# nv-legate/legate.sparse

Hardware: AMD Instinct MI355X
Metric: cg_iters_per_sec (higher is better)
Workload: dtype fp64; 1 GPU; model=poisson2d-5pt-cg, nx=16384, n=268435456, nnz=1342111744, parallelism=dp1 1-D row partition + window gather

## Files before the change

sparse/kernels/__init__.py:

```python
from __future__ import annotations

import os

import torch

_EXT = None
_TRIED = False

_DIR = os.path.dirname(os.path.abspath(__file__))
BUILD_DIR = os.path.join(_DIR, "_build")
SO_PATH = os.path.join(BUILD_DIR, "sparse_hip.so")


def ext():
    global _EXT, _TRIED
    if _EXT is not None or _TRIED:
        return _EXT
    _TRIED = True
    if os.path.exists(SO_PATH):
        torch.ops.load_library(SO_PATH)
        _EXT = torch.ops.sparse_hip
    return _EXT


# ... 324 lines not shown
                     ts._level_ptr, ts._sched, b, x)


def ilu0_factor(fac, values, flag):
    ls = fac._Ls
    ext().ilu0_factor(fac._indptr, fac._indices, values, fac._diag_ptr,
                      ls._order, ls._level_ptr, fac._sched, flag)


_DIA_CONST_DTYPES = (torch.float32, torch.float64)


class DiaMirror:

    __slots__ = ("dvals", "offs", "W", "m", "row0", "off_min", "off_max",
                 "cvals", "mask", "adj")

    def __init__(self, dvals, offs, W, m, row0, off_min=0, off_max=0,
                 cvals=None, mask=None, adj=0):
        self.adj = adj
        self.off_min = off_min
        self.off_max = off_max
        self.dvals = dvals
        self.offs = offs
        self.W = W
        self.m = m
        self.row0 = row0
        self.cvals = cvals
        self.mask = mask

    @property
    def compressed(self) -> bool:
        return self.mask is not None

    def source(self):
        if self.compressed:
            return self.cvals, self.mask
        return self.dvals, None


def build_dia(A, row0: int, compress: bool = True):
    m = A.nrows
    if m == 0 or A.nnz == 0:
        return None
    counts = A.indptr[1:] - A.indptr[:-1]
    rows = torch.repeat_interleave(
        torch.arange(row0, row0 + m, dtype=torch.int64, device=A.device), counts)
    diag = A.indices.long() - rows
    CH = 1 << 30
    if diag.numel() <= CH:
        offs = torch.unique(diag)
    else:
        parts = [torch.unique(diag[i: i + CH])
                 for i in range(0, diag.numel(), CH)]
        offs = torch.unique(torch.cat(parts))
    W = int(offs.numel())
    mp = (m + 1) // 2 * 2
    if W == 0 or W > 48 or W * mp > 1.6 * A.nnz + 4096:
        return None
    need = W * mp * A.values.element_size()
    free, _t = torch.cuda.mem_get_info(A.values.device)
    if need > 0.5 * free:
        return None
    dvals = torch.zeros(W * mp, dtype=A.values.dtype, device=A.device)
    ext().build_dia(A.indptr, A.indices, A.values, offs.contiguous(), dvals,
                    W, int(row0))
    cvals = mask = None
    if (compress and W <= 32 and dvals.dtype in _DIA_CONST_DTYPES
            and os.environ.get("SPARSE_DIA_NOCOMPRESS") != "1"):
        cvals = torch.zeros(W, dtype=dvals.dtype, device=A.device)
        mdt = (torch.uint8 if W <= 8 else
               torch.uint16 if W <= 16 else torch.uint32)
        mask = torch.empty(mp, dtype=mdt, device=A.device)
        ok = torch.ones(1, dtype=torch.int32, device=A.device)
        ext().dia_classify(dvals, cvals, mask, ok, W)
        if int(ok.item()):
            dvals = None
        else:
            cvals = mask = None
    ho = offs.tolist()
    adj = sum(1 << i for i in range(min(W, 32) - 1) if ho[i + 1] == ho[i] + 1)
    return DiaMirror(dvals, offs, W, m, row0, off_min=ho[0], off_max=ho[-1],
                     cvals=cvals, mask=mask, adj=adj)


def _pieces(p):
    hlo, own, hhi = p
    return hlo.contiguous(), own.contiguous(), hhi.contiguous()


def dia_spmv(dm: DiaMirror, pieces, y, col_lo: int, wsize: int,
             rbase: int = 0, rhi: int = -1):
    ext().dia_spmv(*dm.source(), dm.offs, *_pieces(pieces), y, dm.W, dm.m,
                   int(col_lo), dm.row0, int(wsize), int(rbase), int(rhi),
                   dm.adj)


def dia_spmv_dot(dm: DiaMirror, pieces, y, p, col_lo: int, wsize: int,
                 rbase: int = 0, rhi: int = -1):
    return ext().dia_spmv_dot(*dm.source(), dm.offs, *_pieces(pieces), y, p,
                              dm.W, dm.m, int(col_lo), dm.row0, int(wsize),
                              int(rbase), int(rhi), dm.adj)


def dia_spmv_bpdot(dm: DiaMirror, r_pieces, p_pieces, pnew, q,
                   beta_num, beta_den, col_lo: int, wsize: int):
    return ext().dia_spmv_bpdot(*dm.source(), dm.offs, *_pieces(r_pieces),
                                *_pieces(p_pieces), pnew, q, beta_num,
                                beta_den, dm.W, dm.m, int(col_lo), dm.row0,
                                int(wsize), dm.adj)


def cg_xr_norm2(x, p, r, q, a, b, *, nt: int = -1):
    n = x.numel()
    if n == 0:
        return torch.zeros((), dtype=x.dtype, device=x.device)
    ept = max(1, 16 // x.element_size())
    blocks = (n // ept + 255) // 256 + 1
    partial = torch.empty(blocks, dtype=x.dtype, device=x.device)
    ext().cg_xr_norm2(x, p, r, q, a.to(x.dtype), b.to(x.dtype), partial,
                      int(nt))
    return partial.sum()


def dia_residual(dm: DiaMirror, pieces, b, y, col_lo: int, wsize: int,
                 rbase: int = 0, rhi: int = -1):
    ext().dia_residual(*dm.source(), dm.offs, *_pieces(pieces), b, y, dm.W,
                       dm.m, int(col_lo), dm.row0, int(wsize), int(rbase),
                       int(rhi), dm.adj)


def dia_jacobi(dm: DiaMirror, pieces, xloc, b, dinv, omega, xout,
               col_lo: int, wsize: int, rbase: int = 0, rhi: int = -1):
    ext().dia_jacobi(*dm.source(), dm.offs, *_pieces(pieces), xloc, b, dinv,
                     xout, dm.W, dm.m, int(col_lo), dm.row0, int(wsize),
                     float(omega), int(rbase), int(rhi), dm.adj)


class BsrMirror:

    __slots__ = ("bptr", "bcol", "bvals", "nbrows", "m", "fill")

    def __init__(self, bptr, bcol, bvals, nbrows, m, fill):
        self.bptr = bptr
        self.bcol = bcol
        self.bvals = bvals
        self.nbrows = nbrows
        self.m = m
        self.fill = fill


# ... 118 lines not shown
```

sparse/kernels/src/ops.cpp:

```cpp
#include <algorithm>

#include <torch/library.h>

#include <ATen/ATen.h>

void spmv_hip(at::Tensor, at::Tensor, at::Tensor, at::Tensor, at::Tensor,
              int64_t, double);
void spmv_dot_hip(at::Tensor, at::Tensor, at::Tensor, at::Tensor, at::Tensor,
                  at::Tensor, at::Tensor, int64_t);
void axpby_norm2_hip(at::Tensor, at::Tensor, at::Tensor, at::Tensor, bool,
                     bool, at::Tensor);
void build_ell_hip(at::Tensor, at::Tensor, at::Tensor, at::Tensor, at::Tensor,
                   int64_t, int64_t);
void build_dia_hip(at::Tensor, at::Tensor, at::Tensor, at::Tensor, at::Tensor,
                   int64_t, int64_t);
void ell_spmv_plain_hip(at::Tensor, at::Tensor, at::Tensor, at::Tensor,
                        at::Tensor, at::Tensor, int64_t, int64_t, int64_t,
                        int64_t, int64_t);
at::Tensor ell_spmv_dot_hip(at::Tensor, at::Tensor, at::Tensor, at::Tensor,
                            at::Tensor, at::Tensor, at::Tensor, int64_t,
                            int64_t, int64_t, int64_t, int64_t);
void ell_jacobi_hip(at::Tensor, at::Tensor, at::Tensor, at::Tensor,
                    at::Tensor, at::Tensor, at::Tensor, at::Tensor,
                    at::Tensor, int64_t, int64_t, int64_t, double);
void cg_xr_norm2_hip(at::Tensor, at::Tensor, at::Tensor, at::Tensor,
                     at::Tensor, at::Tensor, at::Tensor, int64_t);
using OptTensor = c10::optional<at::Tensor>;
void dia_classify_hip(at::Tensor, at::Tensor, at::Tensor, at::Tensor, int64_t);
at::Tensor dia_spmv_bpdot_hip(at::Tensor, OptTensor, at::Tensor, at::Tensor,
                              at::Tensor, at::Tensor, at::Tensor, at::Tensor,
                              at::Tensor, at::Tensor, at::Tensor, at::Tensor,
                              at::Tensor, int64_t, int64_t, int64_t, int64_t,
                              int64_t, int64_t);
void dia_spmv_plain_hip(at::Tensor, OptTensor, at::Tensor, at::Tensor,
                        at::Tensor, at::Tensor, at::Tensor, int64_t, int64_t,
                        int64_t, int64_t, int64_t, int64_t, int64_t, int64_t);
at::Tensor dia_spmv_dot_hip(at::Tensor, OptTensor, at::Tensor, at::Tensor,
                            at::Tensor, at::Tensor, at::Tensor, at::Tensor,
                            int64_t, int64_t, int64_t, int64_t, int64_t,
                            int64_t, int64_t, int64_t);
void dia_residual_hip(at::Tensor, OptTensor, at::Tensor, at::Tensor,
                      at::Tensor, at::Tensor, at::Tensor, at::Tensor, int64_t,
                      int64_t, int64_t, int64_t, int64_t, int64_t, int64_t,
                      int64_t);
void dia_jacobi_hip(at::Tensor, OptTensor, at::Tensor, at::Tensor, at::Tensor,
                    at::Tensor, at::Tensor, at::Tensor, at::Tensor,
                    at::Tensor, int64_t, int64_t, int64_t, int64_t, int64_t,
                    double, int64_t, int64_t, int64_t);
void add_nnz_hip(at::Tensor, at::Tensor, at::Tensor, at::Tensor, at::Tensor);
void add_compute_hip(at::Tensor, at::Tensor, at::Tensor, at::Tensor, at::Tensor,
                     at::Tensor, at::Tensor, at::Tensor, at::Tensor, double,
                     double);
void mult_nnz_hip(at::Tensor, at::Tensor, at::Tensor, at::Tensor, at::Tensor);
void mult_compute_hip(at::Tensor, at::Tensor, at::Tensor, at::Tensor,
                      at::Tensor, at::Tensor, at::Tensor, at::Tensor,
                      at::Tensor);
void mult_dense_hip(at::Tensor, at::Tensor, at::Tensor, at::Tensor, at::Tensor);
void axpby_hip(at::Tensor, at::Tensor, at::Tensor, at::Tensor, bool, bool,
               int64_t);
void spmm_hip(at::Tensor, at::Tensor, at::Tensor, at::Tensor, at::Tensor,
              int64_t);
void rspmm_hip(at::Tensor, at::Tensor, at::Tensor, at::Tensor, at::Tensor);
void bsr_spmm_hip(at::Tensor, at::Tensor, at::Tensor, at::Tensor, at::Tensor,
// ... 142 lines not shown
        "Tensor(a!) eidx, Tensor(b!) evals, int W, int pad_idx) -> ()");
  m.def("build_dia(Tensor indptr, Tensor indices, Tensor values, "
        "Tensor offs, Tensor(a!) dvals, int W, int row0) -> ()");
  m.def("ell_spmv(Tensor eidx, Tensor evals, Tensor hlo, Tensor own, "
        "Tensor hhi, Tensor(a!) y, int W, int m, int col_lo, "
        "int rbase, int rhi) -> ()");
  m.def("ell_spmv_dot(Tensor eidx, Tensor evals, Tensor hlo, Tensor own, "
        "Tensor hhi, Tensor(a!) y, Tensor pvec, int W, int m, int col_lo, "
        "int rbase, int rhi) -> Tensor");
  m.def("ell_jacobi(Tensor eidx, Tensor evals, Tensor hlo, Tensor own, "
        "Tensor hhi, Tensor xloc, Tensor b, Tensor dinv, Tensor(a!) xout, "
        "int W, int m, int col_lo, float omega) -> ()");
  m.def("cg_xr_norm2(Tensor(a!) x, Tensor p, Tensor(b!) r, Tensor q, "
        "Tensor a, Tensor b, Tensor(c!) dot_out, int nt=-1) -> ()");
  m.def("dia_classify(Tensor dvals, Tensor(a!) cvals, Tensor(b!) mask, "
        "Tensor(c!) ok, int W) -> ()");
  m.def("dia_spmv_bpdot(Tensor planes, Tensor? mask, Tensor offs, "
        "Tensor r_hlo, Tensor r_own, "
        "Tensor r_hhi, Tensor p_hlo, Tensor p_own, Tensor p_hhi, "
        "Tensor(a!) pnew, Tensor(b!) q, Tensor beta_num, Tensor beta_den, "
        "int W, int m, int col_lo, int row0, int wsize, int adj=0) "
        "-> Tensor");
  m.def("dia_spmv(Tensor planes, Tensor? mask, Tensor offs, Tensor hlo, "
        "Tensor own, "
        "Tensor hhi, Tensor(a!) y, int W, int m, int col_lo, int row0, "
        "int wsize, int rbase, int rhi, int adj=0) -> ()");
  m.def("dia_spmv_dot(Tensor planes, Tensor? mask, Tensor offs, Tensor hlo, "
        "Tensor own, "
        "Tensor hhi, Tensor(a!) y, Tensor pvec, int W, int m, int col_lo, "
        "int row0, int wsize, int rbase, int rhi, int adj=0) -> Tensor");
  m.def("dia_residual(Tensor planes, Tensor? mask, Tensor offs, Tensor hlo, "
        "Tensor own, "
        "Tensor hhi, Tensor b, Tensor(a!) y, int W, int m, int col_lo, "
        "int row0, int wsize, int rbase, int rhi, int adj=0) -> ()");
  m.def("dia_jacobi(Tensor planes, Tensor? mask, Tensor offs, Tensor hlo, "
        "Tensor own, "
        "Tensor hhi, Tensor xloc, Tensor b, Tensor dinv, Tensor(a!) xout, "
        "int W, int m, int col_lo, int row0, int wsize, float omega, "
        "int rbase, int rhi, int adj=0) -> ()");
  m.def("spmm(Tensor indptr, Tensor indices, Tensor vals, Tensor B, "
        "Tensor(a!) C, int col_lo) -> ()");
  m.def("rspmm(Tensor indptr, Tensor indices, Tensor vals, Tensor A, "
        "Tensor(a!) C) -> ()");
  m.def("bsr_spmm(Tensor bptr, Tensor bcol, Tensor bvals, Tensor B, "
        "Tensor(a!) C, int col_lo) -> ()");
  m.def("sddmm(Tensor indptr, Tensor indices, Tensor vals, Tensor C, "
        "Tensor D, Tensor(a!) out, int col_lo) -> ()");
  m.def("csr_to_dense(Tensor indptr, Tensor indices, Tensor vals, "
        "Tensor(a!) out) -> ()");
  m.def("coo_to_csr(Tensor rows, Tensor cols, Tensor vals, Tensor(a!) cursor, "
        "Tensor indptr, Tensor(b!) out_idx, Tensor(c!) out_vals, "
        "Tensor(d!) flags) -> ()");
  m.def("dense_to_csr(Tensor D, Tensor(a!) indptr_or_counts, "
        "Tensor(b!) indices, Tensor(c!) vals, bool fill) -> ()");
// ... 70 lines not shown
```

sparse/kernels/src/spmv.hip:

```cpp
#include <type_traits>

#include "common.h"

namespace {

constexpr int BLK = 256;
constexpr int VT = 8;
constexpr int64_t NNZ_PER_BLOCK = (int64_t)BLK * VT;

template <typename U>
struct alignas(4 * sizeof(U) <= 16 ? 4 * sizeof(U) : 16) Quad {
  U v[4];
};

template <typename U>
struct alignas(2 * sizeof(U) <= 16 ? 2 * sizeof(U) : 16) Pair {
  U a, b;
};

template <typename T>
__device__ __forceinline__ void block_reduce_sum(T* red, int tid) {
  __syncthreads();
  for (int w = BLK / 2; w > 0; w >>= 1) {
    if (tid < w) red[tid] += red[tid + w];
// ... 284 lines not shown
  const int64_t r = (int64_t)blockIdx.x * blockDim.x + threadIdx.x;
  if (r >= mp) return;
  uint32_t word = 0;
  bool same = true;
  for (int k = 0; k < W; ++k) {
    const B b = dbits[(int64_t)k * mp + r];
    if (b != 0) {
      word |= 1u << k;
      same = same && b == cbits[k];
    }
  }
  mask[r] = (M)word;
  if (!same && *ok != 0) *ok = 0;
}



template <typename T>
struct XWindow {
  const T* hlo;
  const T* own;
  const T* hhi;
  int64_t nlo, nown, wsize;

  template <bool SINGLE>
  __device__ __forceinline__ T at(int64_t idx) const {
    if (SINGLE) return own[idx];
    if (idx < nlo) return hlo[idx];
    idx -= nlo;
    if (idx < nown) return own[idx];
// ... 77 lines not shown
  __device__ __forceinline__ Rows rows(int64_t r0) const {
    return {dvals + r0, mp};
  }
};

template <int BYTES> struct UIntOf;
template <> struct UIntOf<2> { using type = uint16_t; };
template <> struct UIntOf<4> { using type = uint32_t; };
template <> struct UIntOf<8> { using type = uint64_t; };

template <typename T, typename M>
struct DiaConstPlanes {
  static constexpr int kBatch = 8;
  const T* __restrict__ cvals;
  const M* __restrict__ mask;

  struct Rows {
    const T* __restrict__ c;
    uint32_t m0, m1;
    __device__ __forceinline__ void at(int k, T& v0, T& v1) const {
      const T ck = c[k];
      const uint32_t bit = 1u << k;
      v0 = (m0 & bit) ? ck : T(0);
      v1 = (m1 & bit) ? ck : T(0);
    }
  };
  __device__ __forceinline__ Rows rows(int64_t r0) const {
    using M2 = typename UIntOf<2 * sizeof(M)>::type;
    const M2 w = nt_load(reinterpret_cast<const M2*>(&mask[r0]));
    return {cvals, (uint32_t)(M)w, (uint32_t)(w >> (8 * sizeof(M)))};
// ... 238 lines not shown
  static constexpr int start = ADJ ? __builtin_ctz(ADJ) : 0;
  static constexpr int len = ADJ ? __builtin_popcount(ADJ) + 1 : 1;
  static_assert(ADJ == 0 || (ADJ >> start) + 1 == (1u << (len - 1)),
                "the adjacent diagonals must form one run");
  __host__ __device__ static constexpr DiaSrc src(int P, int i) {
    const int q = i - start;
    if (ADJ == 0 || P < 0 || q < 0 || q >= len) return kDiaLoad;
    if (((P + q) & 1) == 0) return kDiaLoadAligned;
    return q > 0 ? kDiaFromLo : kDiaFromHi;
  }
  __host__ __device__ static constexpr bool two(int P, int i) {
    return src(P, i) == kDiaFromHi && len >= 3;
  }
};

template <int WC, int R, int NWIN, uint32_t ADJ, int P, typename T,
          typename M, typename Comb, typename Pre, typename Post>
__device__ __forceinline__ void dia_const_interior(
    const DiaConstPlanes<T, M>& planes, const int64_t* __restrict__ offs,
    int W, const T* const* own, Comb comb, bool ctr, int64_t rb,
    int64_t cb, int64_t (&o)[WC ? WC : 8], T (&c)[WC ? WC : 8], Pre pre,
    Post post) {
  constexpr int KB = WC ? WC : 8;
  using Run = DiaRun<ADJ>;
  using M2 = typename UIntOf<2 * sizeof(M)>::type;
  const int64_t t2 = 2 * (int64_t)threadIdx.x;
  const int lane = threadIdx.x & 63;
  M2 mw[R];
#pragma unroll
  for (int j = 0; j < R; ++j) {
    mw[j] = nt_load(
        reinterpret_cast<const M2*>(planes.mask + rb + t2 + j * 2 * BLK));
  }
  T a[R][2];
  Pair<T> cx[R];
#pragma unroll
  for (int j = 0; j < R; ++j) {
    a[j][0] = a[j][1] = ZeroOf<T>::value();
    cx[j] = Pair<T>{T(0), T(0)};
  }
  for (int k0 = 0; k0 < W; k0 += KB) {
    if (k0 > 0) {
#pragma unroll
      for (int i = 0; i < KB; ++i) {
        if (k0 + i < W) {
          o[i] = offs[k0 + i];
          c[i] = planes.cvals[k0 + i];
// ... 94 lines not shown
    post(j, rb + t2 + j * 2 * BLK, a[j][0], a[j][1], true, ctr, cx[j]);
  }
}

template <int WC, int R, bool SINGLE, int NWIN, uint32_t ADJ, typename T,
          typename M, typename Comb, typename Pre, typename Post>
__device__ __forceinline__ void dia_const_rows(
    const DiaConstPlanes<T, M>& planes, const int64_t* __restrict__ offs,
    int Wrt, const XWindow<T>& win0, const XWindow<T>& win1, Comb comb,
    const T* rowvec, int64_t m, int64_t row0, int64_t col_lo, int64_t rbase,
    int64_t rhi, Pre pre, Post post) {
  constexpr int KB = WC ? WC : 8;
  constexpr int64_t S = 2 * (int64_t)BLK * R;
  static_assert(ADJ == 0 || (WC > 0 && (ADJ >> (KB - 1)) == 0),
                "a plan needs a compile-time W");
  using Run = DiaRun<ADJ>;
  const int W = WC ? WC : Wrt;
  const int64_t lim = min(m, rhi);
  const int64_t rb = rbase + (int64_t)blockIdx.x * S;
  const int64_t cb = row0 + rb - col_lo - win0.nlo;
  const int64_t own_end = min(win0.nown, win0.wsize - win0.nlo);
  int64_t o[KB];
  T c[KB];
#pragma unroll
  for (int i = 0; i < KB; ++i) {
    if (i < W) {
      o[i] = offs[i];
      c[i] = planes.cvals[i];
    }
  }
  bool interior = rb + S <= lim && cb + o[0] >= 0 &&
                  cb + (S - 1) + (WC ? o[KB - 1] : offs[W - 1]) < own_end;
#pragma unroll
  for (int q = 1; q < Run::len; ++q) {
    interior = interior && o[Run::start + q] == o[Run::start] + q;
  }
  if (interior) {
    const T* own[NWIN];
    own[0] = win0.own;
    own[NWIN - 1] = (NWIN == 2 ? win1 : win0).own;
    const bool ctr = WC > 0 && NWIN == 1 && rowvec != nullptr &&
                     rowvec + rb == win0.own + cb && o[(KB - 1) / 2] == 0;
    auto body = [&](auto par) {
      dia_const_interior<WC, R, NWIN, ADJ, decltype(par)::value>(
          planes, offs, W, own, comb, ctr, rb, cb, o, c, pre, post);
    };
    if (ADJ == 0) {
      body(std::integral_constant<int, -1>{});
    } else {
      const T* u0 = own[0] + (cb + o[Run::start]);
      const T* u1 = own[NWIN - 1] + (cb + o[Run::start]);
      const bool un0 = reinterpret_cast<uintptr_t>(u0) % sizeof(Pair<T>) != 0;
      const bool un1 = reinterpret_cast<uintptr_t>(u1) % sizeof(Pair<T>) != 0;
      if (un0 != un1) {
        body(std::integral_constant<int, -1>{});
      } else if (un0) {
        body(std::integral_constant<int, 1>{});
      } else {
        body(std::integral_constant<int, 0>{});
      }
// ... 14 lines not shown
              for (int w = 0; w < NWIN; ++w) {
                (w == 0 ? win0 : win1)
                    .template pair<SINGLE, true>(c0, v0[w], v1[w]);
              }
              x0 = comb(v0);
              x1 = comb(v1);
            },
            a0, a1);
        post(j, r0, a0, a1, r0 + 1 < lim, false, Pair<T>{T(0), T(0)});
      }
    }
  }
}

template <typename T, typename M, int WC, uint32_t ADJ, bool FUSE_DOT,
          bool SINGLE, bool RESID>
__global__ __launch_bounds__(BLK) void dia_const_spmv_kernel(
    const DiaConstPlanes<T, M> planes, const int64_t* __restrict__ offs,
    const XWindow<T> win, T* __restrict__ y, const T* __restrict__ pvec,
    T* __restrict__ dot_partial, int64_t m, int W, int64_t col_lo,
    int64_t row0, int64_t rbase, int64_t rhi) {
  constexpr int R = dia_spmv_pairs(WC, RESID);
  const int64_t lim = min(m, rhi);
  Pair<T> pv[R];
  T d[R];
#pragma unroll
  for (int j = 0; j < R; ++j) {
    pv[j] = Pair<T>{T(0), T(0)};
    d[j] = T(0);
  }
  dia_const_rows<WC, R, SINGLE, 1, ADJ>(
// ... 3 lines not shown
        if ((FUSE_DOT || RESID) && !ctr) {
          if (full) {
            pv[j] = *reinterpret_cast<const Pair<T>*>(&pvec[r0]);
          } else if (r0 < lim) {
            pv[j].a = pvec[r0];
          }
        }
      },
      [&](int j, int64_t r0, T a0, T a1, bool full, bool ctr, Pair<T> cx) {
        if (ctr) pv[j] = cx;
        if (RESID) {
          a0 = pv[j].a - a0;
          a1 = pv[j].b - a1;
        }
        if (full) {
          *reinterpret_cast<Pair<T>*>(&y[r0]) = Pair<T>{a0, a1};
        } else {
          store_pair_or_tail(y, r0, m, rhi, a0, a1);
        }
        if (FUSE_DOT) {
          T dd = T(0);
          if (full || r0 < lim) dd = fmadd(a0, pv[j].a, dd);
          if (full) dd = fmadd(a1, pv[j].b, dd);
          d[j] = dd;
        }
      });
  if (FUSE_DOT) {
    const T sum = block_sums_256<R>(d);
    const int64_t slot = (int64_t)blockIdx.x * R + threadIdx.x;
    if (threadIdx.x < R && slot * (2 * BLK) < rhi - rbase) {
      dot_partial[slot] = sum;
// ... 113 lines not shown

  template <int R, typename... P, typename... A>
  void launch_pairs(void (*kern)(P...), A... args) const {
    hipLaunchKernelGGL(kern, dim3((nblocks + R - 1) / R), dim3(BLK), 0,
                       cur_stream(), static_cast<P>(args)...);
  }
};

using OptTensor = c10::optional<at::Tensor>;

inline int64_t dia_mp(const at::Tensor& planes, const OptTensor& mask,
                      int64_t W) {
  return mask ? mask->numel() : planes.numel() / W;
}

template <typename T, typename F>
void dispatch_dia_planes(const at::Tensor& planes, const OptTensor& mask,
                         int64_t W, F&& f) {
  if (!mask) {
    f(DiaPlanes<T>{planes.data_ptr<T>(), planes.numel() / W});
    return;
  }
  if constexpr (std::is_floating_point_v<T>) {
    TORCH_CHECK(planes.numel() == W && W <= 8 * (int64_t)mask->element_size() &&
                    mask->numel() % 2 == 0,
                "dia: W constants and an even number of mask words of at "
                "least W bits expected");
    const T* c = planes.data_ptr<T>();
    const void* mw = mask->data_ptr();
    switch (mask->scalar_type()) {
      case at::kByte:
        f(DiaConstPlanes<T, uint8_t>{c, static_cast<const uint8_t*>(mw)});
        return;
      case at::kUInt16:
        f(DiaConstPlanes<T, uint16_t>{c, static_cast<const uint16_t*>(mw)});
        return;
      case at::kUInt32:
        f(DiaConstPlanes<T, uint32_t>{c, static_cast<const uint32_t*>(mw)});
        return;
      default:
        break;
    }
  }
  TORCH_CHECK(false, "dia: constant planes need a real value type and a "
                     "uint8/uint16/uint32 row mask");
}

template <typename P>
struct DiaConstOf : std::false_type {};
template <typename T, typename M>
struct DiaConstOf<DiaConstPlanes<T, M>> : std::true_type {
  using mask_t = M;
};
// ... 20 lines not shown

template <typename M, typename F>
void dispatch_dia_wc(int64_t W, int64_t adj, F&& f) {
  TORCH_CHECK(W >= 1, "dia: at least one diagonal expected");
  if constexpr (std::is_same_v<M, uint8_t>) {
    switch (W) {
#define SPARSE_DIA_WC(N) \
  case N: dispatch_dia_adj<N>(adj, f); return;
      SPARSE_DIA_WC(1) SPARSE_DIA_WC(2) SPARSE_DIA_WC(3) SPARSE_DIA_WC(4)
      SPARSE_DIA_WC(5) SPARSE_DIA_WC(6) SPARSE_DIA_WC(7) SPARSE_DIA_WC(8)
#undef SPARSE_DIA_WC
      default: break;
    }
  }
  f(std::integral_constant<int, 0>{}, std::integral_constant<uint32_t, 0>{});
}

}

void build_ell_hip(at::Tensor indptr, at::Tensor indices, at::Tensor values,
                   at::Tensor eidx, at::Tensor evals, int64_t W,
                   int64_t pad_idx) {
  const int64_t m = indptr.numel() - 1;
  const int64_t mp = evals.numel() / W;
  DISPATCH_VALUES(values.scalar_type(), "build_ell", [&] {
    using T = scalar_t;
    DISPATCH_INDEX(indices.scalar_type(), "build_ell_idx", [&] {
      hipLaunchKernelGGL((build_ell_kernel<T, index_t>), dim3((mp + 255) / 256),
                         dim3(256), 0, cur_stream(), indptr.data_ptr<int64_t>(),
                         indices.data_ptr<index_t>(), values.data_ptr<T>(),
// ... 11 lines not shown
  if (m == 0) return;
  DISPATCH_VALUES(values.scalar_type(), "build_dia", [&] {
    using T = scalar_t;
    DISPATCH_INDEX(indices.scalar_type(), "build_dia_idx", [&] {
      hipLaunchKernelGGL((build_dia_kernel<T, index_t>),
                         dim3((m + 255) / 256), dim3(256), 0, cur_stream(),
                         indptr.data_ptr<int64_t>(),
                         indices.data_ptr<index_t>(), values.data_ptr<T>(),
                         offs.data_ptr<int64_t>(), dvals.data_ptr<T>(), m, mp,
                         (int)W, row0);
    });
  });
}

void dia_classify_hip(at::Tensor dvals, at::Tensor cvals, at::Tensor mask,
                      at::Tensor ok, int64_t W) {
  const int64_t mp = mask.numel();
  TORCH_CHECK(dvals.numel() == W * mp && cvals.numel() == W &&
                  cvals.scalar_type() == dvals.scalar_type() &&
                  ok.scalar_type() == at::kInt &&
                  W <= 8 * (int64_t)mask.element_size(),
              "dia_classify: inconsistent arguments");
  if (mp == 0) return;
  const dim3 g1((unsigned)std::min<int64_t>((mp + 255) / 256, 1024),
                (unsigned)W);
  auto run = [&](auto bits, auto word) {
    using B = decltype(bits);
    using M = decltype(word);
    const B* d = static_cast<const B*>(dvals.data_ptr());
    B* c = static_cast<B*>(cvals.data_ptr());
    hipLaunchKernelGGL((dia_plane_const_kernel<B>), g1, dim3(256), 0,
                       cur_stream(), d, c, mp);
    hipLaunchKernelGGL((dia_row_mask_kernel<B, M>), dim3((mp + 255) / 256),
                       dim3(256), 0, cur_stream(), d, c,
                       static_cast<M*>(mask.data_ptr()),
                       ok.data_ptr<int32_t>(), mp, (int)W);
  };
  auto by_word = [&](auto bits) {
    switch (mask.scalar_type()) {
      case at::kByte: run(bits, uint8_t{}); break;
      case at::kUInt16: run(bits, uint16_t{}); break;
      case at::kUInt32: run(bits, uint32_t{}); break;
      default: TORCH_CHECK(false, "dia_classify: mask must be uint8/16/32");
    }
  };
  switch (dvals.scalar_type()) {
    case at::kFloat: by_word(uint32_t{}); break;
    case at::kDouble: by_word(uint64_t{}); break;
    default: TORCH_CHECK(false, "dia_classify: fp32/fp64 planes only");
  }
}
// ... 63 lines not shown
                 L.window<T>(hlo, own, hhi), xloc.data_ptr<T>(),
                 b.data_ptr<T>(), dinv.data_ptr<T>(), xout.data_ptr<T>(), m,
                 L.mp, W, col_lo, omega);
      });
    });
  });
}

template <bool RESID>
static at::Tensor dia_spmv_impl(const at::Tensor& planes, const OptTensor& mask,
                                const at::Tensor& offs, const at::Tensor& hlo,
                                const at::Tensor& own, const at::Tensor& hhi,
                                at::Tensor& y, const at::Tensor* pvec,
                                int64_t W, int64_t m, int64_t col_lo,
                                int64_t row0, int64_t wsize, int64_t rbase,
                                int64_t rhi, int64_t adj) {
  const RowPairLaunch L(dia_mp(planes, mask, W), hlo, own, hhi, wsize, rbase,
                        rhi);
  const bool fuse_dot = pvec && !RESID;
  at::Tensor partial;
  if (L.empty()) return partial;
  if (fuse_dot) partial = at::empty({L.nblocks}, planes.options());
  DISPATCH_VALUES(planes.scalar_type(), "dia_spmv", [&] {
    using T = scalar_t;
    dispatch_dia_planes<T>(planes, mask, W, [&](auto pl) {
      dispatch_bool(fuse_dot, [&](auto fuse) {
        dispatch_bool(L.single, [&](auto single) {
          using PL = decltype(pl);
          const T* pp = pvec ? pvec->data_ptr<T>() : nullptr;
          T* dp = fuse_dot ? partial.data_ptr<T>() : nullptr;
          if constexpr (RESID && decltype(fuse)::value) {
          } else if constexpr (DiaConstOf<PL>::value) {
            using M = typename DiaConstOf<PL>::mask_t;
            dispatch_dia_wc<M>(W, adj, [&](auto wc, auto plan) {
              L.launch_pairs<dia_spmv_pairs(decltype(wc)::value, RESID)>(
                  dia_const_spmv_kernel<T, M, decltype(wc)::value,
                                        decltype(plan)::value,
                                        decltype(fuse)::value,
                                        decltype(single)::value, RESID>,
                  pl, offs.data_ptr<int64_t>(), L.window<T>(hlo, own, hhi),
                  y.data_ptr<T>(), pp, dp, m, W, col_lo, row0, L.rbase,
                  L.rhi);
            });
          } else {
            L.launch(dia_spmv_kernel<T, PL, decltype(fuse)::value,
                                     decltype(single)::value, RESID>,
                     pl, offs.data_ptr<int64_t>(), L.window<T>(hlo, own, hhi),
                     y.data_ptr<T>(), pp, dp, m, L.mp, W, col_lo, row0,
                     L.rbase, L.rhi);
          }
        });
      });
    });
  });
  return partial;
}

void dia_spmv_plain_hip(at::Tensor planes, OptTensor mask, at::Tensor offs,
                        at::Tensor hlo, at::Tensor own, at::Tensor hhi,
                        at::Tensor y, int64_t W, int64_t m, int64_t col_lo,
                        int64_t row0, int64_t wsize, int64_t rbase,
                        int64_t rhi, int64_t adj) {
  dia_spmv_impl<false>(planes, mask, offs, hlo, own, hhi, y, nullptr, W, m,
                       col_lo, row0, wsize, rbase, rhi, adj);
}

at::Tensor dia_spmv_dot_hip(at::Tensor planes, OptTensor mask, at::Tensor offs,
                            at::Tensor hlo, at::Tensor own, at::Tensor hhi,
                            at::Tensor y, at::Tensor pvec, int64_t W,
                            int64_t m, int64_t col_lo, int64_t row0,
                            int64_t wsize, int64_t rbase, int64_t rhi,
                            int64_t adj) {
  return sum_or_zero(dia_spmv_impl<false>(planes, mask, offs, hlo, own, hhi, y,
                                          &pvec, W, m, col_lo, row0, wsize,
                                          rbase, rhi, adj),
                     planes);
}

void dia_residual_hip(at::Tensor planes, OptTensor mask, at::Tensor offs,
                      at::Tensor hlo, at::Tensor own, at::Tensor hhi,
                      at::Tensor b, at::Tensor y, int64_t W, int64_t m,
                      int64_t col_lo, int64_t row0, int64_t wsize,
                      int64_t rbase, int64_t rhi, int64_t adj) {
  dia_spmv_impl<true>(planes, mask, offs, hlo, own, hhi, y, &b, W, m, col_lo,
                      row0, wsize, rbase, rhi, adj);
}

void dia_jacobi_hip(at::Tensor planes, OptTensor mask, at::Tensor offs,
                    at::Tensor hlo, at::Tensor own, at::Tensor hhi,
                    at::Tensor xloc, at::Tensor b, at::Tensor dinv,
                    at::Tensor xout, int64_t W, int64_t m, int64_t col_lo,
                    int64_t row0, int64_t wsize, double omega, int64_t rbase,
                    int64_t rhi, int64_t adj) {
  const RowPairLaunch L(dia_mp(planes, mask, W), hlo, own, hhi, wsize, rbase,
                        rhi);
  if (L.empty()) return;
  DISPATCH_VALUES(planes.scalar_type(), "dia_jacobi", [&] {
    using T = scalar_t;
    dispatch_dia_planes<T>(planes, mask, W, [&](auto pl) {
      dispatch_bool(L.single, [&](auto single) {
        using PL = decltype(pl);
        if constexpr (DiaConstOf<PL>::value) {
          using M = typename DiaConstOf<PL>::mask_t;
          dispatch_dia_wc<M>(W, adj, [&](auto wc, auto plan) {
            L.launch_pairs<kDiaSmoothPairs>(
                dia_const_jacobi_kernel<T, M, decltype(wc)::value,
                                        decltype(plan)::value,
                                        decltype(single)::value>,
                pl, offs.data_ptr<int64_t>(), L.window<T>(hlo, own, hhi),
                xloc.data_ptr<T>(), b.data_ptr<T>(), dinv.data_ptr<T>(),
                xout.data_ptr<T>(), m, W, col_lo, row0, omega, L.rbase,
                L.rhi);
          });
        } else {
// ... 3 lines not shown
                   xout.data_ptr<T>(), m, L.mp, W, col_lo, row0, omega,
                   L.rbase, L.rhi);
        }
      });
    });
  });
}

at::Tensor dia_spmv_bpdot_hip(at::Tensor planes, OptTensor mask,
                              at::Tensor offs, at::Tensor r_hlo,
                              at::Tensor r_own, at::Tensor r_hhi,
                              at::Tensor p_hlo, at::Tensor p_own,
                              at::Tensor p_hhi, at::Tensor pnew, at::Tensor q,
                              at::Tensor beta_num, at::Tensor beta_den,
                              int64_t W, int64_t m, int64_t col_lo,
                              int64_t row0, int64_t wsize, int64_t adj) {
  TORCH_CHECK(pnew.data_ptr() != p_own.data_ptr(),
              "dia_spmv_bpdot: pnew must not alias p_own (double-buffer)");
  const RowPairLaunch L(dia_mp(planes, mask, W), r_hlo, r_own, r_hhi, wsize);
  at::Tensor partial;
  if (L.empty()) return sum_or_zero(partial, planes);
  partial = at::empty({L.nblocks}, planes.options());
  DISPATCH_VALUES(planes.scalar_type(), "dia_spmv_bpdot", [&] {
    using T = scalar_t;
    dispatch_dia_planes<T>(planes, mask, W, [&](auto pl) {
      dispatch_bool(L.single, [&](auto single) {
        using PL = decltype(pl);
        auto go = [&](auto launch, auto kern) {
          launch(kern, pl, offs.data_ptr<int64_t>(),
                 L.window<T>(r_hlo, r_own, r_hhi),
                 L.window<T>(p_hlo, p_own, p_hhi), pnew.data_ptr<T>(),
                 q.data_ptr<T>(), beta_num.data_ptr<T>(),
                 beta_den.data_ptr<T>(), partial.data_ptr<T>(), m, L.mp, W,
                 col_lo, row0);
        };
        if constexpr (DiaConstOf<PL>::value) {
          using M = typename DiaConstOf<PL>::mask_t;
          dispatch_dia_wc<M>(W, adj, [&](auto wc, auto plan) {
            go([&](auto... a) { L.launch_pairs<kDiaBpdotPairs>(a...); },
               dia_const_bpdot_kernel<T, M, decltype(wc)::value,
// ... 13 lines not shown
```

Baseline: 258.5 iters/s.

## Skip DIA mask loads for all-full slices and add nontemporal y stores

Adds a per-512-row slice flag array, built at classify time, that marks slices whose compressed-DIA mask is all ones. Interior kernels use it to skip the per-row mask loads for those slices, which cuts mask traffic on the Poisson stencil where nearly all rows are full. It also adds an optional nontemporal store path for the SpMV output, enabled automatically for vectors of 256 MiB or more on uint8-mask, small-W variants. This costs extra kernel instantiations and a small flag read per block, and nontemporal stores could hurt if y is reread soon afterwards.

```diff
diff --git a/sparse/kernels/__init__.py b/sparse/kernels/__init__.py
--- a/sparse/kernels/__init__.py
+++ b/sparse/kernels/__init__.py
@@ -362,11 +362,13 @@
 class DiaMirror:
 
     __slots__ = ("dvals", "offs", "W", "m", "row0", "off_min", "off_max",
-                 "cvals", "mask", "adj")
+                 "cvals", "mask", "adj", "flags", "use_flags")
 
     def __init__(self, dvals, offs, W, m, row0, off_min=0, off_max=0,
-                 cvals=None, mask=None, adj=0):
+                 cvals=None, mask=None, adj=0, flags=None):
         self.adj = adj
+        self.flags = flags
+        self.use_flags = True
         self.off_min = off_min
         self.off_max = off_max
         self.dvals = dvals
@@ -385,6 +387,9 @@
         if self.compressed:
             return self.cvals, self.mask
         return self.dvals, None
+
+    def slice_flags(self):
+        return self.flags if self.use_flags and self.compressed else None
 
 
 def build_dia(A, row0: int, compress: bool = True):
@@ -413,7 +418,7 @@
     dvals = torch.zeros(W * mp, dtype=A.values.dtype, device=A.device)
     ext().build_dia(A.indptr, A.indices, A.values, offs.contiguous(), dvals,
                     W, int(row0))
-    cvals = mask = None
+    cvals = mask = flags = None
     if (compress and W <= 32 and dvals.dtype in _DIA_CONST_DTYPES
             and os.environ.get("SPARSE_DIA_NOCOMPRESS") != "1"):
         cvals = torch.zeros(W, dtype=dvals.dtype, device=A.device)
@@ -421,15 +426,17 @@
                torch.uint16 if W <= 16 else torch.uint32)
         mask = torch.empty(mp, dtype=mdt, device=A.device)
         ok = torch.ones(1, dtype=torch.int32, device=A.device)
-        ext().dia_classify(dvals, cvals, mask, ok, W)
+        flags = torch.zeros(4 * ((mp + 511) // 512 // 4 + 2),
+                            dtype=torch.uint8, device=A.device)
+        ext().dia_classify(dvals, cvals, mask, ok, W, flags, m)
         if int(ok.item()):
             dvals = None
         else:
-            cvals = mask = None
+            cvals = mask = flags = None
     ho = offs.tolist()
     adj = sum(1 << i for i in range(min(W, 32) - 1) if ho[i + 1] == ho[i] + 1)
     return DiaMirror(dvals, offs, W, m, row0, off_min=ho[0], off_max=ho[-1],
-                     cvals=cvals, mask=mask, adj=adj)
+                     cvals=cvals, mask=mask, adj=adj, flags=flags)
 
 
 def _pieces(p):
@@ -438,17 +445,18 @@
 
 
 def dia_spmv(dm: DiaMirror, pieces, y, col_lo: int, wsize: int,
-             rbase: int = 0, rhi: int = -1):
+             rbase: int = 0, rhi: int = -1, *, nt: int = -1):
     ext().dia_spmv(*dm.source(), dm.offs, *_pieces(pieces), y, dm.W, dm.m,
                    int(col_lo), dm.row0, int(wsize), int(rbase), int(rhi),
-                   dm.adj)
+                   dm.adj, dm.slice_flags(), int(nt))
 
 
 def dia_spmv_dot(dm: DiaMirror, pieces, y, p, col_lo: int, wsize: int,
-                 rbase: int = 0, rhi: int = -1):
+                 rbase: int = 0, rhi: int = -1, *, nt: int = -1):
     return ext().dia_spmv_dot(*dm.source(), dm.offs, *_pieces(pieces), y, p,
                               dm.W, dm.m, int(col_lo), dm.row0, int(wsize),
-                              int(rbase), int(rhi), dm.adj)
+                              int(rbase), int(rhi), dm.adj, dm.slice_flags(),
+                              int(nt))
 
 
 def dia_spmv_bpdot(dm: DiaMirror, r_pieces, p_pieces, pnew, q,
@@ -456,7 +464,7 @@
     return ext().dia_spmv_bpdot(*dm.source(), dm.offs, *_pieces(r_pieces),
                                 *_pieces(p_pieces), pnew, q, beta_num,
                                 beta_den, dm.W, dm.m, int(col_lo), dm.row0,
-                                int(wsize), dm.adj)
+                                int(wsize), dm.adj, dm.slice_flags())
 
 
 def cg_xr_norm2(x, p, r, q, a, b, *, nt: int = -1):
@@ -475,14 +483,14 @@
                  rbase: int = 0, rhi: int = -1):
     ext().dia_residual(*dm.source(), dm.offs, *_pieces(pieces), b, y, dm.W,
                        dm.m, int(col_lo), dm.row0, int(wsize), int(rbase),
-                       int(rhi), dm.adj)
+                       int(rhi), dm.adj, None)
 
 
 def dia_jacobi(dm: DiaMirror, pieces, xloc, b, dinv, omega, xout,
                col_lo: int, wsize: int, rbase: int = 0, rhi: int = -1):
     ext().dia_jacobi(*dm.source(), dm.offs, *_pieces(pieces), xloc, b, dinv,
                      xout, dm.W, dm.m, int(col_lo), dm.row0, int(wsize),
-                     float(omega), int(rbase), int(rhi), dm.adj)
+                     float(omega), int(rbase), int(rhi), dm.adj, None)
 
 
 class BsrMirror:
diff --git a/sparse/kernels/src/ops.cpp b/sparse/kernels/src/ops.cpp
--- a/sparse/kernels/src/ops.cpp
+++ b/sparse/kernels/src/ops.cpp
@@ -26,27 +26,29 @@
 void cg_xr_norm2_hip(at::Tensor, at::Tensor, at::Tensor, at::Tensor,
                      at::Tensor, at::Tensor, at::Tensor, int64_t);
 using OptTensor = c10::optional<at::Tensor>;
-void dia_classify_hip(at::Tensor, at::Tensor, at::Tensor, at::Tensor, int64_t);
+void dia_classify_hip(at::Tensor, at::Tensor, at::Tensor, at::Tensor, int64_t,
+                      OptTensor, int64_t);
 at::Tensor dia_spmv_bpdot_hip(at::Tensor, OptTensor, at::Tensor, at::Tensor,
                               at::Tensor, at::Tensor, at::Tensor, at::Tensor,
                               at::Tensor, at::Tensor, at::Tensor, at::Tensor,
                               at::Tensor, int64_t, int64_t, int64_t, int64_t,
-                              int64_t, int64_t);
+                              int64_t, int64_t, OptTensor);
 void dia_spmv_plain_hip(at::Tensor, OptTensor, at::Tensor, at::Tensor,
                         at::Tensor, at::Tensor, at::Tensor, int64_t, int64_t,
-                        int64_t, int64_t, int64_t, int64_t, int64_t, int64_t);
+                        int64_t, int64_t, int64_t, int64_t, int64_t, int64_t,
+                        OptTensor, int64_t);
 at::Tensor dia_spmv_dot_hip(at::Tensor, OptTensor, at::Tensor, at::Tensor,
                             at::Tensor, at::Tensor, at::Tensor, at::Tensor,
                             int64_t, int64_t, int64_t, int64_t, int64_t,
-                            int64_t, int64_t, int64_t);
+                            int64_t, int64_t, int64_t, OptTensor, int64_t);
 void dia_residual_hip(at::Tensor, OptTensor, at::Tensor, at::Tensor,
                       at::Tensor, at::Tensor, at::Tensor, at::Tensor, int64_t,
                       int64_t, int64_t, int64_t, int64_t, int64_t, int64_t,
-                      int64_t);
+                      int64_t, OptTensor);
 void dia_jacobi_hip(at::Tensor, OptTensor, at::Tensor, at::Tensor, at::Tensor,
                     at::Tensor, at::Tensor, at::Tensor, at::Tensor,
                     at::Tensor, int64_t, int64_t, int64_t, int64_t, int64_t,
-                    double, int64_t, int64_t, int64_t);
+                    double, int64_t, int64_t, int64_t, OptTensor);
 void add_nnz_hip(at::Tensor, at::Tensor, at::Tensor, at::Tensor, at::Tensor);
 void add_compute_hip(at::Tensor, at::Tensor, at::Tensor, at::Tensor, at::Tensor,
                      at::Tensor, at::Tensor, at::Tensor, at::Tensor, double,
@@ -219,30 +221,33 @@
   m.def("cg_xr_norm2(Tensor(a!) x, Tensor p, Tensor(b!) r, Tensor q, "
         "Tensor a, Tensor b, Tensor(c!) dot_out, int nt=-1) -> ()");
   m.def("dia_classify(Tensor dvals, Tensor(a!) cvals, Tensor(b!) mask, "
-        "Tensor(c!) ok, int W) -> ()");
+        "Tensor(c!) ok, int W, Tensor(d!)? flags=None, int m=-1) -> ()");
   m.def("dia_spmv_bpdot(Tensor planes, Tensor? mask, Tensor offs, "
         "Tensor r_hlo, Tensor r_own, "
         "Tensor r_hhi, Tensor p_hlo, Tensor p_own, Tensor p_hhi, "
         "Tensor(a!) pnew, Tensor(b!) q, Tensor beta_num, Tensor beta_den, "
-        "int W, int m, int col_lo, int row0, int wsize, int adj=0) "
-        "-> Tensor");
+        "int W, int m, int col_lo, int row0, int wsize, int adj=0, "
+        "Tensor? flags=None) -> Tensor");
   m.def("dia_spmv(Tensor planes, Tensor? mask, Tensor offs, Tensor hlo, "
         "Tensor own, "
         "Tensor hhi, Tensor(a!) y, int W, int m, int col_lo, int row0, "
-        "int wsize, int rbase, int rhi, int adj=0) -> ()");
+        "int wsize, int rbase, int rhi, int adj=0, Tensor? flags=None, "
+        "int nt=-1) -> ()");
   m.def("dia_spmv_dot(Tensor planes, Tensor? mask, Tensor offs, Tensor hlo, "
         "Tensor own, "
         "Tensor hhi, Tensor(a!) y, Tensor pvec, int W, int m, int col_lo, "
-        "int row0, int wsize, int rbase, int rhi, int adj=0) -> Tensor");
+        "int row0, int wsize, int rbase, int rhi, int adj=0, "
+        "Tensor? flags=None, int nt=-1) -> Tensor");
   m.def("dia_residual(Tensor planes, Tensor? mask, Tensor offs, Tensor hlo, "
         "Tensor own, "
         "Tensor hhi, Tensor b, Tensor(a!) y, int W, int m, int col_lo, "
-        "int row0, int wsize, int rbase, int rhi, int adj=0) -> ()");
+        "int row0, int wsize, int rbase, int rhi, int adj=0, "
+        "Tensor? flags=None) -> ()");
   m.def("dia_jacobi(Tensor planes, Tensor? mask, Tensor offs, Tensor hlo, "
         "Tensor own, "
         "Tensor hhi, Tensor xloc, Tensor b, Tensor dinv, Tensor(a!) xout, "
         "int W, int m, int col_lo, int row0, int wsize, float omega, "
-        "int rbase, int rhi, int adj=0) -> ()");
+        "int rbase, int rhi, int adj=0, Tensor? flags=None) -> ()");
   m.def("spmm(Tensor indptr, Tensor indices, Tensor vals, Tensor B, "
         "Tensor(a!) C, int col_lo) -> ()");
   m.def("rspmm(Tensor indptr, Tensor indices, Tensor vals, Tensor A, "
diff --git a/sparse/kernels/src/spmv.hip b/sparse/kernels/src/spmv.hip
--- a/sparse/kernels/src/spmv.hip
+++ b/sparse/kernels/src/spmv.hip
@@ -322,6 +322,20 @@
   if (!same && *ok != 0) *ok = 0;
 }
 
+constexpr int kDiaCell = 512;
+
+template <typename M>
+__global__ __launch_bounds__(kDiaCell / 2) void dia_slice_flags_kernel(
+    const M* __restrict__ mask, uint8_t* __restrict__ flags, int64_t m,
+    int W) {
+  const int64_t r = (int64_t)blockIdx.x * kDiaCell + 2 * threadIdx.x;
+  const uint32_t full = W >= 32 ? 0xffffffffu : (1u << W) - 1u;
+  const bool ok = r + 1 < m && (uint32_t)mask[r] == full &&
+                  (uint32_t)mask[r + 1] == full;
+  const int all = __syncthreads_and(ok);
+  if (threadIdx.x == 0) flags[blockIdx.x] = all ? 1 : 0;
+}
+
 
 
 template <typename T>
@@ -429,6 +443,7 @@
   static constexpr int kBatch = 8;
   const T* __restrict__ cvals;
   const M* __restrict__ mask;
+  const uint32_t* __restrict__ flags = nullptr;
 
   struct Rows {
     const T* __restrict__ c;
@@ -697,13 +712,26 @@
   }
 };
 
+template <bool NT, typename T>
+__device__ __forceinline__ void pair_store(T* p, const Pair<T>& v) {
+  if constexpr (NT && std::is_arithmetic_v<T>) {
+    typedef unsigned int bits_t
+        __attribute__((ext_vector_type(sizeof(Pair<T>) / 4)));
+    bits_t t;
+    __builtin_memcpy(&t, &v, sizeof(v));
+    __builtin_nontemporal_store(t, reinterpret_cast<bits_t*>(p));
+  } else {
+    *reinterpret_cast<Pair<T>*>(p) = v;
+  }
+}
+
 template <int WC, int R, int NWIN, uint32_t ADJ, int P, typename T,
           typename M, typename Comb, typename Pre, typename Post>
 __device__ __forceinline__ void dia_const_interior(
     const DiaConstPlanes<T, M>& planes, const int64_t* __restrict__ offs,
     int W, const T* const* own, Comb comb, bool ctr, int64_t rb,
-    int64_t cb, int64_t (&o)[WC ? WC : 8], T (&c)[WC ? WC : 8], Pre pre,
-    Post post) {
+    int64_t cb, uint32_t uni, int64_t (&o)[WC ? WC : 8],
+    T (&c)[WC ? WC : 8], Pre pre, Post post) {
   constexpr int KB = WC ? WC : 8;
   using Run = DiaRun<ADJ>;
   using M2 = typename UIntOf<2 * sizeof(M)>::type;
@@ -712,8 +740,11 @@
   M2 mw[R];
 #pragma unroll
   for (int j = 0; j < R; ++j) {
-    mw[j] = nt_load(
-        reinterpret_cast<const M2*>(planes.mask + rb + t2 + j * 2 * BLK));
+    mw[j] = ~M2(0);
+    if (!(uni >> j & 1)) {
+      mw[j] = nt_load(
+          reinterpret_cast<const M2*>(planes.mask + rb + t2 + j * 2 * BLK));
+    }
   }
   T a[R][2];
   Pair<T> cx[R];
@@ -838,6 +869,8 @@
   constexpr int64_t S = 2 * (int64_t)BLK * R;
   static_assert(ADJ == 0 || (WC > 0 && (ADJ >> (KB - 1)) == 0),
                 "a plan needs a compile-time W");
+  static_assert(2 * BLK == kDiaCell && R <= 4,
+                "a slice is one flag cell wide; R + 1 cells fit two dwords");
   using Run = DiaRun<ADJ>;
   const int W = WC ? WC : Wrt;
   const int64_t lim = min(m, rhi);
@@ -853,6 +886,20 @@
       c[i] = planes.cvals[i];
     }
   }
+  uint32_t uni = 0;
+  if (planes.flags != nullptr) {
+    const int64_t c0 = rb / kDiaCell;
+    const uint64_t fw = (planes.flags[c0 / 4] |
+                         (uint64_t)planes.flags[c0 / 4 + 1] << 32) >>
+                        (8 * (c0 % 4));
+    const bool split = rb % kDiaCell != 0;
+#pragma unroll
+    for (int j = 0; j < R; ++j) {
+      const bool here = (fw >> (8 * j) & 0xff) != 0;
+      const bool next = (fw >> (8 * j + 8) & 0xff) != 0;
+      if (here && (!split || next)) uni |= 1u << j;
+    }
+  }
   bool interior = rb + S <= lim && cb + o[0] >= 0 &&
                   cb + (S - 1) + (WC ? o[KB - 1] : offs[W - 1]) < own_end;
 #pragma unroll
@@ -867,7 +914,7 @@
                      rowvec + rb == win0.own + cb && o[(KB - 1) / 2] == 0;
     auto body = [&](auto par) {
       dia_const_interior<WC, R, NWIN, ADJ, decltype(par)::value>(
-          planes, offs, W, own, comb, ctr, rb, cb, o, c, pre, post);
+          planes, offs, W, own, comb, ctr, rb, cb, uni, o, c, pre, post);
     };
     if (ADJ == 0) {
       body(std::integral_constant<int, -1>{});
@@ -912,7 +959,7 @@
 }
 
 template <typename T, typename M, int WC, uint32_t ADJ, bool FUSE_DOT,
-          bool SINGLE, bool RESID>
+          bool SINGLE, bool RESID, bool NT_STORE = false>
 __global__ __launch_bounds__(BLK) void dia_const_spmv_kernel(
     const DiaConstPlanes<T, M> planes, const int64_t* __restrict__ offs,
     const XWindow<T> win, T* __restrict__ y, const T* __restrict__ pvec,
@@ -946,7 +993,7 @@
           a1 = pv[j].b - a1;
         }
         if (full) {
-          *reinterpret_cast<Pair<T>*>(&y[r0]) = Pair<T>{a0, a1};
+          pair_store<NT_STORE>(&y[r0], Pair<T>{a0, a1});
         } else {
           store_pair_or_tail(y, r0, m, rhi, a0, a1);
         }
@@ -1090,9 +1137,24 @@
   return mask ? mask->numel() : planes.numel() / W;
 }
 
+inline int64_t dia_flag_bytes(int64_t mp) {
+  return 4 * ((mp + kDiaCell - 1) / kDiaCell / 4 + 2);
+}
+
+inline const uint32_t* dia_flag_words(const OptTensor& flags, int64_t rhi) {
+  if (!flags) return nullptr;
+  TORCH_CHECK(flags->scalar_type() == at::kByte && flags->is_contiguous() &&
+                  flags->numel() >= dia_flag_bytes(rhi) &&
+                  reinterpret_cast<uintptr_t>(flags->data_ptr()) % 4 == 0,
+              "dia: slice flags must be ", dia_flag_bytes(rhi),
+              " contiguous, dword-aligned uint8 for ", rhi, " rows");
+  return static_cast<const uint32_t*>(flags->data_ptr());
+}
+
 template <typename T, typename F>
 void dispatch_dia_planes(const at::Tensor& planes, const OptTensor& mask,
-                         int64_t W, F&& f) {
+                         const OptTensor& flags, int64_t rhi, int64_t W,
+                         F&& f) {
   if (!mask) {
     f(DiaPlanes<T>{planes.data_ptr<T>(), planes.numel() / W});
     return;
@@ -1104,15 +1166,18 @@
                 "least W bits expected");
     const T* c = planes.data_ptr<T>();
     const void* mw = mask->data_ptr();
+    const uint32_t* fl = dia_flag_words(flags, rhi);
     switch (mask->scalar_type()) {
       case at::kByte:
-        f(DiaConstPlanes<T, uint8_t>{c, static_cast<const uint8_t*>(mw)});
+        f(DiaConstPlanes<T, uint8_t>{c, static_cast<const uint8_t*>(mw), fl});
         return;
       case at::kUInt16:
-        f(DiaConstPlanes<T, uint16_t>{c, static_cast<const uint16_t*>(mw)});
+        f(DiaConstPlanes<T, uint16_t>{c, static_cast<const uint16_t*>(mw),
+                                      fl});
         return;
       case at::kUInt32:
-        f(DiaConstPlanes<T, uint32_t>{c, static_cast<const uint32_t*>(mw)});
+        f(DiaConstPlanes<T, uint32_t>{c, static_cast<const uint32_t*>(mw),
+                                      fl});
         return;
       default:
         break;
@@ -1163,6 +1228,19 @@
     }
   }
   f(std::integral_constant<int, 0>{}, std::integral_constant<uint32_t, 0>{});
+}
+
+constexpr int64_t kDiaNtMinBytes = int64_t(256) << 20;
+
+inline bool dia_nt_mode(int64_t nt, int64_t vec_bytes) {
+  TORCH_CHECK(nt >= -1 && nt <= 1, "dia_spmv: nt must be -1, 0 or 1, got ",
+              nt);
+  return nt >= 0 ? nt == 1 : vec_bytes >= kDiaNtMinBytes;
+}
+
+template <typename M>
+constexpr bool dia_nt_built(int WC, bool resid) {
+  return std::is_same_v<M, uint8_t> && !resid && WC >= 1 && WC <= 5;
 }
 
 }
@@ -1204,13 +1282,16 @@
 }
 
 void dia_classify_hip(at::Tensor dvals, at::Tensor cvals, at::Tensor mask,
-                      at::Tensor ok, int64_t W) {
+                      at::Tensor ok, int64_t W, OptTensor flags, int64_t m) {
   const int64_t mp = mask.numel();
   TORCH_CHECK(dvals.numel() == W * mp && cvals.numel() == W &&
                   cvals.scalar_type() == dvals.scalar_type() &&
                   ok.scalar_type() == at::kInt &&
                   W <= 8 * (int64_t)mask.element_size(),
               "dia_classify: inconsistent arguments");
+  TORCH_CHECK(!flags || (m >= 0 && m <= mp && mp % 2 == 0),
+              "dia_classify: slice flags need m <= mp rows, mp even");
+  if (flags) dia_flag_words(flags, mp);
   if (mp == 0) return;
   const dim3 g1((unsigned)std::min<int64_t>((mp + 255) / 256, 1024),
                 (unsigned)W);
@@ -1225,6 +1306,12 @@
                        dim3(256), 0, cur_stream(), d, c,
                        static_cast<M*>(mask.data_ptr()),
                        ok.data_ptr<int32_t>(), mp, (int)W);
+    if (flags && m >= kDiaCell) {
+      hipLaunchKernelGGL((dia_slice_flags_kernel<M>), dim3(m / kDiaCell),
+                         dim3(kDiaCell / 2), 0, cur_stream(),
+                         static_cast<const M*>(mask.data_ptr()),
+                         flags->data_ptr<uint8_t>(), m, (int)W);
+    }
   };
   auto by_word = [&](auto bits) {
     switch (mask.scalar_type()) {
@@ -1318,16 +1405,18 @@
                                 at::Tensor& y, const at::Tensor* pvec,
                                 int64_t W, int64_t m, int64_t col_lo,
                                 int64_t row0, int64_t wsize, int64_t rbase,
-                                int64_t rhi, int64_t adj) {
+                                int64_t rhi, int64_t adj,
+                                const OptTensor& flags, int64_t nt) {
   const RowPairLaunch L(dia_mp(planes, mask, W), hlo, own, hhi, wsize, rbase,
                         rhi);
   const bool fuse_dot = pvec && !RESID;
+  const bool nt_store = dia_nt_mode(nt, y.numel() * y.element_size());
   at::Tensor partial;
   if (L.empty()) return partial;
   if (fuse_dot) partial = at::empty({L.nblocks}, planes.options());
   DISPATCH_VALUES(planes.scalar_type(), "dia_spmv", [&] {
     using T = scalar_t;
-    dispatch_dia_planes<T>(planes, mask, W, [&](auto pl) {
+    dispatch_dia_planes<T>(planes, mask, flags, L.rhi, W, [&](auto pl) {
       dispatch_bool(fuse_dot, [&](auto fuse) {
         dispatch_bool(L.single, [&](auto single) {
           using PL = decltype(pl);
@@ -1337,14 +1426,18 @@
           } else if constexpr (DiaConstOf<PL>::value) {
             using M = typename DiaConstOf<PL>::mask_t;
             dispatch_dia_wc<M>(W, adj, [&](auto wc, auto plan) {
-              L.launch_pairs<dia_spmv_pairs(decltype(wc)::value, RESID)>(
-                  dia_const_spmv_kernel<T, M, decltype(wc)::value,
-                                        decltype(plan)::value,
-                                        decltype(fuse)::value,
-                                        decltype(single)::value, RESID>,
-                  pl, offs.data_ptr<int64_t>(), L.window<T>(hlo, own, hhi),
-                  y.data_ptr<T>(), pp, dp, m, W, col_lo, row0, L.rbase,
-                  L.rhi);
+              constexpr int WC = decltype(wc)::value;
+              constexpr bool built = dia_nt_built<M>(WC, RESID);
+              dispatch_bool(built && nt_store, [&](auto nts) {
+                L.launch_pairs<dia_spmv_pairs(WC, RESID)>(
+                    dia_const_spmv_kernel<T, M, WC, decltype(plan)::value,
+                                          decltype(fuse)::value,
+                                          decltype(single)::value, RESID,
+                                          built && decltype(nts)::value>,
+                    pl, offs.data_ptr<int64_t>(), L.window<T>(hlo, own, hhi),
+                    y.data_ptr<T>(), pp, dp, m, W, col_lo, row0, L.rbase,
+                    L.rhi);
+              });
             });
           } else {
             L.launch(dia_spmv_kernel<T, PL, decltype(fuse)::value,
@@ -1364,9 +1457,10 @@
                         at::Tensor hlo, at::Tensor own, at::Tensor hhi,
                         at::Tensor y, int64_t W, int64_t m, int64_t col_lo,
                         int64_t row0, int64_t wsize, int64_t rbase,
-                        int64_t rhi, int64_t adj) {
+                        int64_t rhi, int64_t adj, OptTensor flags,
+                        int64_t nt) {
   dia_spmv_impl<false>(planes, mask, offs, hlo, own, hhi, y, nullptr, W, m,
-                       col_lo, row0, wsize, rbase, rhi, adj);
+                       col_lo, row0, wsize, rbase, rhi, adj, flags, nt);
 }
 
 at::Tensor dia_spmv_dot_hip(at::Tensor planes, OptTensor mask, at::Tensor offs,
@@ -1374,10 +1468,10 @@
                             at::Tensor y, at::Tensor pvec, int64_t W,
                             int64_t m, int64_t col_lo, int64_t row0,
                             int64_t wsize, int64_t rbase, int64_t rhi,
-                            int64_t adj) {
+                            int64_t adj, OptTensor flags, int64_t nt) {
   return sum_or_zero(dia_spmv_impl<false>(planes, mask, offs, hlo, own, hhi, y,
                                           &pvec, W, m, col_lo, row0, wsize,
-                                          rbase, rhi, adj),
+                                          rbase, rhi, adj, flags, nt),
                      planes);
 }
 
@@ -1385,9 +1479,10 @@
                       at::Tensor hlo, at::Tensor own, at::Tensor hhi,
                       at::Tensor b, at::Tensor y, int64_t W, int64_t m,
                       int64_t col_lo, int64_t row0, int64_t wsize,
-                      int64_t rbase, int64_t rhi, int64_t adj) {
+                      int64_t rbase, int64_t rhi, int64_t adj,
+                      OptTensor flags) {
   dia_spmv_impl<true>(planes, mask, offs, hlo, own, hhi, y, &b, W, m, col_lo,
-                      row0, wsize, rbase, rhi, adj);
+                      row0, wsize, rbase, rhi, adj, flags, 0);
 }
 
 void dia_jacobi_hip(at::Tensor planes, OptTensor mask, at::Tensor offs,
@@ -1395,13 +1490,13 @@
                     at::Tensor xloc, at::Tensor b, at::Tensor dinv,
                     at::Tensor xout, int64_t W, int64_t m, int64_t col_lo,
                     int64_t row0, int64_t wsize, double omega, int64_t rbase,
-                    int64_t rhi, int64_t adj) {
+                    int64_t rhi, int64_t adj, OptTensor flags) {
   const RowPairLaunch L(dia_mp(planes, mask, W), hlo, own, hhi, wsize, rbase,
                         rhi);
   if (L.empty()) return;
   DISPATCH_VALUES(planes.scalar_type(), "dia_jacobi", [&] {
     using T = scalar_t;
-    dispatch_dia_planes<T>(planes, mask, W, [&](auto pl) {
+    dispatch_dia_planes<T>(planes, mask, flags, L.rhi, W, [&](auto pl) {
       dispatch_bool(L.single, [&](auto single) {
         using PL = decltype(pl);
         if constexpr (DiaConstOf<PL>::value) {
@@ -1435,7 +1530,8 @@
                               at::Tensor p_hhi, at::Tensor pnew, at::Tensor q,
                               at::Tensor beta_num, at::Tensor beta_den,
                               int64_t W, int64_t m, int64_t col_lo,
-                              int64_t row0, int64_t wsize, int64_t adj) {
+                              int64_t row0, int64_t wsize, int64_t adj,
+                              OptTensor flags) {
   TORCH_CHECK(pnew.data_ptr() != p_own.data_ptr(),
               "dia_spmv_bpdot: pnew must not alias p_own (double-buffer)");
   const RowPairLaunch L(dia_mp(planes, mask, W), r_hlo, r_own, r_hhi, wsize);
@@ -1444,7 +1540,7 @@
   partial = at::empty({L.nblocks}, planes.options());
   DISPATCH_VALUES(planes.scalar_type(), "dia_spmv_bpdot", [&] {
     using T = scalar_t;
-    dispatch_dia_planes<T>(planes, mask, W, [&](auto pl) {
+    dispatch_dia_planes<T>(planes, mask, flags, L.mp, W, [&](auto pl) {
       dispatch_bool(L.single, [&](auto single) {
         using PL = decltype(pl);
         auto go = [&](auto launch, auto kern) {
```

Result: no change. 260.8 iters/s (median of 6 runs) (+0.9%).
